# dan-lee-gh/monte-carlo-gp

Measured on AMD Instinct MI355X. Metric: race-simulations/sec (20 drivers, 60 laps), higher is better.
Workload: dtype f64

## Files before the change

### monte_carlo_gp_amd/csrc/mcgp_hip.hip

```cpp
#include "../../include/mcgp.h"
#include "params_build.h"
#include "race_kernel.hip.h"
#include "race_kernel_reg.hip.h"
#include "championship.hip.h"
#include "matchups.hip.h"
#include "resume.hip.h"

#define MCGP_FE_FN __host__ __device__ static inline
#include "frontend_exp.h"
#include "elo_update.h"
#include "normal53_table.h"

#include <hip/hip_runtime.h>

#include <cmath>
#include <cstdio>
#include <cstdlib>
#include <algorithm>
#include <cstring>
#include <mutex>
#include <new>
#include <string>
#include <vector>

// ... 191 lines not shown
    c.champ_keys_bytes = c.champ_bytes = 0;
    if (c.d_match) (void)hipFree(c.d_match);
    c.d_match = nullptr;
    c.match_bytes = 0;
    if (c.d_resume) (void)hipFree(c.d_resume);
    c.d_resume = nullptr;
    c.resume_bytes = 0;
    c.batch_bytes = c.batch_retire_bytes = 0;
    for (auto &t : c.timer) {
        if (t.start) (void)hipEventDestroy(t.start);
        if (t.stop) (void)hipEventDestroy(t.stop);
        if (t.d_ticket) (void)hipFree(t.d_ticket);
        if (t.d_retire) (void)hipFree(t.d_retire);
        t = DeviceCtx::Timer{};
    }
    c.last_timer = -1;
    c.d_hist = nullptr;
    c.d_grid = c.d_order1 = c.d_orders = nullptr;
    c.d_orders_bytes = 0;
}

int init_ctx_body(int device, DeviceCtx &c)
{
    HIP_TRY(hipSetDevice(device));
    hipDeviceProp_t prop;
    HIP_TRY(hipGetDeviceProperties(&prop, device));
    c.cu_count = prop.multiProcessorCount;
    c.lds_per_block = prop.sharedMemPerBlock;
    if (const char *e = std::getenv("MCGP_LDS_PER_BLOCK")) {
        const unsigned long long v = std::strtoull(e, nullptr, 10);
        if (v >= 16384 && v < c.lds_per_block) c.lds_per_block = (size_t)v;
    }
    for (auto &sl : c.slot) {
        HIP_TRY(hipMalloc(&sl.dev, sizeof(mcgp::KParams)));
        HIP_TRY(hipHostMalloc(&sl.host, sizeof(mcgp::KParams)));
        HIP_TRY(hipEventCreateWithFlags(&sl.uploaded, hipEventDisableTiming));
    }
    HIP_TRY(hipMalloc(&c.d_hist, sizeof(unsigned long long) * MCGP_MAX_CARS * MCGP_MAX_CARS));
    HIP_TRY(hipMalloc(&c.d_grid, MCGP_MAX_CARS));
    HIP_TRY(hipMalloc(&c.d_order1, MCGP_MAX_CARS));
    HIP_TRY(hipMalloc(&c.d_fe_in, sizeof(double) * 4 * MCGP_MAX_CARS));
    HIP_TRY(hipMalloc(&c.d_fe_pen, sizeof(int32_t) * MCGP_MAX_CARS));
    HIP_TRY(hipMalloc(&c.d_fe_out, sizeof(double) * MCGP_MAX_CARS * MCGP_MAX_CARS));
    HIP_TRY(hipMalloc(&c.d_norm53, sizeof(mcgp_normal53_table_bits)));
    HIP_TRY(hipMemcpy(c.d_norm53, mcgp_normal53_table_bits, sizeof(mcgp_normal53_table_bits), hipMemcpyHostToDevice));
    HIP_TRY(hipFuncSetAttribute(reinterpret_cast<const void *>(&mcgp::race_kernel),
                                hipFuncAttributeMaxDynamicSharedMemorySize, (int)c.lds_per_block));
    HIP_TRY(hipFuncSetAttribute(reinterpret_cast<const void *>(&mcgp::race_resume_kernel),
                                hipFuncAttributeMaxDynamicSharedMemorySize, (int)c.lds_per_block));
    return MCGP_OK;
}

int ensure_ctx_locked(int device, DeviceCtx &c)
{
    if (c.ready) return MCGP_OK;
    const int rc = init_ctx_body(device, c);
    if (rc != MCGP_OK) {
        release_ctx(c);
        return rc;
    }
    c.ready = true;
    return MCGP_OK;
}

int build_params(const mcgp_config *cfg, const mcgp_drivers *drv, const double *grid_probs, uint32_t n,
                 mcgp::KParams *kp)
{
    const char *err = "";
// ... 51 lines not shown
        MCGP_REG_SIZES(X)
#undef X
        default: return nullptr;
    }
}

KernelFn select_small_kernel(uint32_t n)
{
    switch (n) {
#define X(N_) case N_: return &mcgp::race_kernel_reg<N_, mcgp::kSmallBlockWaves>;
        MCGP_REG_SIZES(X)
#undef X
        default: return nullptr;
    }
}

KernelFn select_kernel(const mcgp::KParams &kp, bool *is_reg)
{
    *is_reg = false;
    const uint32_t n = (uint32_t)kp.n;
    const char *force = std::getenv("MCGP_FORCE_GENERIC");
    if (force && force[0] == '1') return &mcgp::race_kernel;
    if (!mcgp::reg_kernel_serves(kp)) return &mcgp::race_kernel;
    switch (n) {
#define X(N_) case N_: *is_reg = true; return &mcgp::race_kernel_reg<N_>;
        MCGP_REG_SIZES(X)
#undef X
        default: return &mcgp::race_kernel;
    }
}

void launch_geometry(const DeviceCtx &c, uint32_t n, bool is_reg, KernelFn kernel, uint64_t n_sims, uint32_t *grid,
                     uint32_t *block, uint32_t *lds, int reg_waves = 0 ,
                     bool wide = false , int total_laps = 0)
{
    int reg_cap = 8;
    {
        hipFuncAttributes attr;
        if (hipFuncGetAttributes(&attr, reinterpret_cast<const void *>(kernel)) == hipSuccess && attr.numRegs > 0) {
            const int alloc = ((attr.numRegs + 7) / 8) * 8;
            int per_simd = 512 / alloc;
            if (per_simd > 8) per_simd = 8;
            if (per_simd < 1) per_simd = 1;
            reg_cap = 4 * per_simd;
        }
    }
    int waves = 1, blocks_per_cu = 1;
    size_t bytes = 0;
    if (is_reg) {
        waves = reg_waves ? reg_waves : mcgp::reg_block_waves((int)n);
        bytes = wide ? mcgp::wide_launch_lds_bytes((int)n, waves, total_laps)
                     : mcgp::shared_lds_bytes_reg((int)n) + (size_t)waves * 64 * mcgp::per_thread_lds_bytes_reg((int)n);
    } else {
        const size_t per_wave = 64 * mcgp::per_thread_lds_bytes((int)n);
        waves = (int)((c.lds_per_block - mcgp::kSharedTableBytes) / per_wave);
        if (waves > 8) waves = 8;
        if (waves < 1) waves = 1;
        uint32_t threads = (uint32_t)waves * 64u;
        if (n_sims < threads) threads = (uint32_t)(((n_sims + 63) / 64) * 64);
        if (threads == 0) threads = 64;
        waves = (int)(threads / 64);
        bytes = mcgp::kSharedTableBytes + (size_t)threads * mcgp::per_thread_lds_bytes((int)n);
    }
    blocks_per_cu = (int)(c.lds_per_block / bytes);
    if (blocks_per_cu * waves > reg_cap) blocks_per_cu = reg_cap / waves;
    if (blocks_per_cu < 1) blocks_per_cu = 1;
    const uint32_t threads = (uint32_t)waves * 64u;
    const uint64_t n_batches = (n_sims + threads - 1) / threads;
    uint64_t g = (uint64_t)c.cu_count * (uint64_t)blocks_per_cu;
    if (g > n_batches) g = n_batches;
    if (g < 1) g = 1;
    *grid = (uint32_t)g;
    *block = threads;
    *lds = (uint32_t)bytes;
}

uint64_t max_sims_per_launch()
{
    uint64_t cap = 0xFFFFFE00ull;
    if (const char *e = std::getenv("MCGP_MAX_SIMS_PER_LAUNCH")) {
        const unsigned long long v = std::strtoull(e, nullptr, 10);
        if (v >= 1 && v < cap) cap = v;
    }
    return cap;
// ... 56 lines not shown

int launch(DeviceCtx &c, const mcgp::KParams &kp, uint64_t n_sims, uint64_t sim_offset, uint64_t seed,
           hipStream_t stream, unsigned long long *d_hist, uint8_t *d_orders, const uint8_t *d_fixed_grid,
           const FrontEnd &fe = FrontEnd())
{
    if (n_sims == 0) return MCGP_OK;
    bool is_reg = false;
    KernelFn kernel = select_kernel(kp, &is_reg);
    WideKernelFn wide = nullptr;
    if (kp.wide) {
        wide = select_wide_kernel((uint32_t)kp.n);
        if (!wide || !mcgp::reg_kernel_serves(kp))
            return fail(MCGP_E_BAD_ARG, "deviates = MCGP_DEVIATES_53 serves the problems the register kernel takes "
                                        "(reg_kernel_serves: lap times clear of zero, overtake_delta >= 0)");
        HIP_TRY(hipFuncSetAttribute(reinterpret_cast<const void *>(wide), hipFuncAttributeMaxDynamicSharedMemorySize,
                                    (int)c.lds_per_block));
        is_reg = true;
        kernel = nullptr;
    }
    DeviceCtx::Slot *sl = nullptr;
    if (!fe.on)
        for (auto &cand : c.slot)
            if (cand.used && cand.shareable && std::memcmp(cand.host, &kp, sizeof(kp)) == 0) { sl = &cand; break; }
    if (!sl) {
        sl = &c.slot[c.next_slot];
        c.next_slot = (c.next_slot + 1) % kParamSlots;
        if (sl->used)
            for (auto &rd : sl->reader)
                if (rd.live) {
                    HIP_TRY(hipEventSynchronize(rd.done));
                    rd.live = false;
                }
        std::memcpy(sl->host, &kp, sizeof(kp));
        sl->used = true;
        sl->shareable = !fe.on;
        HIP_TRY(hipMemcpyAsync(sl->dev, sl->host, sizeof(kp), hipMemcpyHostToDevice, stream));
        if (fe.on) {
            hipLaunchKernelGGL(grid_probs_kernel, dim3(1), dim3(mcgp::kMaxCars), 0, stream, c.d_fe_in, c.d_fe_pen,
                               (int)kp.n, sl->dev->grid_probs);
            HIP_TRY(hipGetLastError());
        }
        HIP_TRY(hipEventRecord(sl->uploaded, stream));
        sl->upload_stream = stream;
    } else if (sl->upload_stream != stream) {
        HIP_TRY(hipStreamWaitEvent(stream, sl->uploaded, 0));
    }
    int ti = -1;
    {
        const int rc = claim_timer(c, stream, &ti);
        if (rc != MCGP_OK) return rc;
    }
    c.timer[ti].seq = ++c.timer_seq;
    if (!c.timer[ti].d_ticket) return fail(MCGP_E_HIP, "no work counter for this stream");
    HIP_TRY(hipEventRecord(c.timer[ti].start, stream));
    const uint64_t cap = max_sims_per_launch();
    uint32_t grid = 0, block = 0, lds = 0;
    bool small_shape = false;
    auto resource_error = [](hipError_t e) {
        return e == hipErrorOutOfMemory || e == hipErrorInvalidValue || e == hipErrorLaunchOutOfResources ||
               e == hipErrorInvalidConfiguration;
    };
    for (uint64_t done = 0; done < n_sims; done += cap) {
        const uint64_t m = (n_sims - done) < cap ? (n_sims - done) : cap;
        for (;;) {
            KernelFn k = kernel;
            if (small_shape) {
                k = select_small_kernel((uint32_t)kp.n);
                if (!k) return fail(MCGP_E_HIP, "no small-block instantiation for this field size");
            }
            launch_geometry(c, (uint32_t)kp.n, is_reg, wide ? reinterpret_cast<KernelFn>(wide) : k, m, &grid, &block, &lds,
                            wide ? mcgp::wide_block_waves(kp.n) : small_shape ? mcgp::kSmallBlockWaves : 0, wide != nullptr,
                            kp.total_laps);
            const bool may_shrink = is_reg && !wide && !small_shape;
            if (may_shrink && lds > c.lds_per_block) {
                small_shape = true;
                continue;
            }
            if (lds > c.lds_per_block)
                return fail(MCGP_E_HIP, "the kernel's smallest block needs " + std::to_string(lds) + " bytes of LDS, the device offers " +
                                            std::to_string(c.lds_per_block) + " per block");
            if (is_reg && !wide) {
                const hipError_t e = hipFuncSetAttribute(reinterpret_cast<const void *>(k),
                                                         hipFuncAttributeMaxDynamicSharedMemorySize, (int)lds);
                if (e != hipSuccess) {
                    (void)hipGetLastError();
                    if (may_shrink && resource_error(e)) { small_shape = true; continue; }
                    return fail(MCGP_E_HIP, std::string("hipFuncSetAttribute(dynamic LDS): ") + hipGetErrorString(e));
                }
            }
            const uint64_t unit = is_reg ? 64u : block;
            const uint64_t n_batches = (m + unit - 1) / unit;
            if (is_reg) {
                HIP_TRY(hipMemsetAsync(c.timer[ti].d_ticket, 0, sizeof(uint32_t), stream));
                const size_t want = mcgp::reg_retire_ws_bytes(kp.n, (size_t)grid * block);
                if (want > c.timer[ti].retire_bytes) {
                    if (c.timer[ti].d_retire) {
                        HIP_TRY(hipStreamSynchronize(stream));
                        (void)hipFree(c.timer[ti].d_retire);
                    }
                    c.timer[ti].d_retire = nullptr;
                    c.timer[ti].retire_bytes = 0;
                    HIP_TRY(hipMalloc(&c.timer[ti].d_retire, want));
                    c.timer[ti].retire_bytes = want;
                }
            }
// ... 942 lines not shown
```

### monte_carlo_gp_amd/csrc/params_build.h

```cpp
#pragma once
#include "../../include/mcgp.h"
#include "normal_table.h"
#include "race_common.hip.h"

#include <cmath>
#include <cstring>

namespace mcgp {

inline uint64_t threshold(double p)
{
    if (!(p > 0.0)) return 0;
    const double x = p * 4294967296.0;
    if (x >= 4294967296.0) return 4294967296ull;
    return (uint64_t)std::ceil(x);
}

inline uint64_t threshold53(double p)
{
    if (!(p > 0.0)) return 0;
    const double x = p * 9007199254740992.0;
    if (x >= 9007199254740992.0) return 9007199254740992ull;
    return (uint64_t)std::ceil(x);
}
// ... 48 lines not shown
        if (cfg->comp_optimal_laps[c] < 0 || cfg->comp_optimal_laps[c] > 50000)
            { *err = "comp_optimal_laps out of range"; return MCGP_E_BAD_ARG; }
    }
    for (uint32_t d = 0; d < n; ++d) {
        const double deg = drv->tire_deg[d];
        kp->base_pace[d] = drv->base_pace[d];
        kp->factor[d] = deg > 0 ? deg / 0.05 : 1.0;
        kp->tire_deg[d] = deg;
        kp->variance[d] = drv->variance[d];
        kp->t_dnf1[d] = threshold(drv->team_dnf[d] * 4.0);
        kp->t_dnf[d] = threshold(drv->lap_dnf[d]);
        kp->t53_dnf1[d] = threshold53(drv->team_dnf[d] * 4.0);
        kp->q64_dnf[d] = survival64(drv->lap_dnf[d]);
        const double pit_deg = drv->tire_deg_pit[d];
        for (int c = 0; c < 5; ++c) {
            int opt = cfg->comp_optimal_laps[c];
            if (pit_deg > 0.05) opt = (int)((double)opt * 0.85);
            else if (pit_deg < 0.02) opt = (int)((double)opt * 1.1);
            kp->opt_laps[d * kCompStride + c] = (uint16_t)opt;
        }
    }
    if (grid_probs)
        for (uint32_t d = 0; d < n; ++d)
            for (uint32_t s = 0; s < n; ++s) {
                const double p = grid_probs[(size_t)d * n + s];
                if (!(p >= 0.0)) { *err = "grid_probs has a negative or NaN entry"; return MCGP_E_BAD_ARG; }
                kp->grid_probs[(size_t)d * n + s] = p;
            }
    static_assert(sizeof(mcgp_normal_table_bits) == sizeof(kp->normal_bits), "normal table size");
    std::memcpy(kp->normal_bits, mcgp_normal_table_bits, sizeof(kp->normal_bits));
    return MCGP_OK;
}

}
```

### monte_carlo_gp_amd/csrc/race_common.hip.h

```cpp
#pragma once
#include <hip/hip_runtime.h>
#include <stdint.h>

namespace mcgp {

constexpr int kMaxCars = 32;
constexpr int kNormalRows = 448;
constexpr int kNormal53Rows = 784;
constexpr int kNormal53RowBytes = 64;
constexpr int kCompStride = 8;

constexpr uint32_t kPurposeGrid = 0u << 16;
constexpr uint32_t kPurposeEvent = 1u << 16;
constexpr uint32_t kPurposeCar = 2u << 16;
constexpr uint32_t kPurposeOvt = 3u << 16;
constexpr uint32_t kPurposeRetire = 4u << 16;

__host__ __device__ inline uint32_t retire_next_threshold(uint32_t S, uint32_t q)
{
    return (uint32_t)(((uint64_t)S * (uint64_t)q) >> 32);
}
__host__ __device__ inline uint32_t draw_retirement_lap(uint32_t w, uint64_t t, int L)
{
    if (t == 0ull) return 0u;
// ... 1 lines not shown
    uint32_t S = q;
    for (int k = 2; k <= L; ++k) {
        if (!(w < S)) return (uint32_t)k;
        S = retire_next_threshold(S, q);
    }
    return 0u;
}
__host__ __device__ inline uint32_t draw_retirement_lap_after(uint32_t w, uint64_t t, int k, int L)
{
    const uint32_t r = draw_retirement_lap(w, t, L - k + 1);
    return r == 0u ? 0u : (uint32_t)(k - 1) + r;
}

struct KParams {
    int32_t n, total_laps, track, pop_sh, pop_mh, pad0;
    double pit_loss, overtake_delta, drs_delta, dirty_thr, dirty_pen;
    double overtake_delta_31;
    uint64_t t_red, t_sc, t_vsc, t_vsc_tire;
    double comp_deg[kCompStride], comp_delta[kCompStride];
    double base_pace[kMaxCars];
    double factor[kMaxCars];
    double tire_deg[kMaxCars];
    double variance[kMaxCars];
    uint64_t t_dnf1[kMaxCars];
    uint64_t t_dnf[kMaxCars];
    uint16_t opt_laps[kMaxCars * kCompStride];
    double grid_probs[kMaxCars * kMaxCars];
    uint32_t normal_bits[kNormalRows * 4];
    int32_t wide, pad1;
    uint64_t t53_red, t53_sc, t53_vsc, t53_vsc_tire;
    uint64_t t53_dnf1[kMaxCars];
    uint64_t q64_dnf[kMaxCars];
};

constexpr size_t kSharedTableBytes =
    kNormalRows * 16
    + 4 * kMaxCars * 8
    + 2 * kMaxCars * 8
    + kMaxCars * kCompStride * 2
    + 2 * kCompStride * 8
    + kMaxCars * kMaxCars * 4;
__host__ __device__ constexpr size_t per_thread_lds_bytes(int n) { return (size_t)n * (8 + 8 + 4 + 1 + 2); }

__device__ __forceinline__ uint32_t xor3_key(uint32_t a, uint32_t b, uint32_t key)
{
#if defined(__HIP_DEVICE_COMPILE__)
    uint32_t r;
    asm("v_bitop3_b32 %0, %1, %2, %3 bitop3:0x96" : "=v"(r) : "v"(a), "v"(b), "s"(key));
    return r;
#else
    return a ^ b ^ key;
#endif
}

__device__ __forceinline__ void philox4x32_10(uint32_t c0, uint32_t c1, uint32_t c2, uint32_t c3,
                                              uint32_t k0, uint32_t k1,
                                              uint32_t &o0, uint32_t &o1, uint32_t &o2, uint32_t &o3)
{
#pragma unroll
    for (int r = 0; r < 10; ++r) {
        const uint64_t p0 = (uint64_t)0xD2511F53u * c0;
        const uint64_t p1 = (uint64_t)0xCD9E8D57u * c2;
        const uint32_t n0 = xor3_key((uint32_t)(p1 >> 32), c1, k0);
        const uint32_t n2 = xor3_key((uint32_t)(p0 >> 32), c3, k1);
        c1 = (uint32_t)p1;
        c3 = (uint32_t)p0;
// ... 93 lines not shown
```

### monte_carlo_gp_amd/csrc/race_isa.hip.h

```cpp
#ifndef MCGP_RACE_ISA_H
#define MCGP_RACE_ISA_H
#include <hip/hip_runtime.h>

namespace mcgp {

__device__ __forceinline__ void minmax_f64(double a, double b, double &lo, double &hi)
{
    asm("v_min_f64 %0, %1, %2" : "=v"(lo) : "v"(a), "v"(b));
    asm("v_max_f64 %0, %1, %2" : "=v"(hi) : "v"(a), "v"(b));
}

__device__ __forceinline__ double max_f64(double a, double b)
{
    double r;
    asm("v_max_f64 %0, %1, %2" : "=v"(r) : "v"(a), "v"(b));
    return r;
}

__device__ __forceinline__ double max_abs_f64(double a, double b)
{
    double r;
    asm("v_max_f64 %0, |%1|, %2" : "=v"(r) : "v"(a), "v"(b));
    return r;
}
// ... 223 lines not shown
            "v_ceil_f64 %[t], %[dl]\n\t"
            "v_cvt_u32_f64 %[thr], %[t]\n\t"
            "v_min_u32 %[thr], 0x80000000, %[thr]\n\t"
            "v_add_u32 %[next], %[stride], %[row]\n\t"
            "v_cndmask_b32 %[thr], 0, %[thr], vcc\n\t"
            "v_cndmask_b32 %[next], %[row], %[next], vcc"
            : [t] "=&v"(t), [thr] "=&v"(thr), [next] "=&v"(next)
            : [dl] "v"(dl), [od] "s"(od), [row] "v"(row), [stride] "n"(STRIDE)
            : "vcc");
    } else {
        asm("v_cmp_lt_f64 vcc, %[od], %[dl]\n\t"
            "v_cvt_u32_f64 %[thr], %[dl]\n\t"
            "v_add_u32 %[next], %[stride], %[row]\n\t"
            "v_min_u32 %[thr], 0x80000000, %[thr]\n\t"
            "v_cndmask_b32 %[next], %[row], %[next], vcc\n\t"
            "v_cndmask_b32 %[thr], 0, %[thr], vcc"
            : [thr] "=&v"(thr), [next] "=&v"(next)
            : [dl] "v"(dl), [od] "s"(od), [row] "v"(row), [stride] "n"(STRIDE)
            : "vcc");
    }
}

#define MCGP_LDS __attribute__((address_space(3)))
template <typename T>
__device__ __forceinline__ T lds_ld(uint32_t addr)
{
    return *reinterpret_cast<const MCGP_LDS T *>(addr);
}
template <typename T>
__device__ __forceinline__ void lds_st(uint32_t addr, T v)
{
    *reinterpret_cast<MCGP_LDS T *>(addr) = v;
}
__device__ __forceinline__ void lds_or_u32(uint32_t addr, uint32_t bits)
{
    (void)__hip_atomic_fetch_or(reinterpret_cast<MCGP_LDS uint32_t *>(addr), bits, __ATOMIC_RELAXED, __HIP_MEMORY_SCOPE_WAVEFRONT);
}
__device__ __forceinline__ float4 lds_ld_float4(uint32_t addr)
{
    typedef float v4f __attribute__((ext_vector_type(4)));
    const v4f v = *reinterpret_cast<const MCGP_LDS v4f *>(addr);
    return make_float4(v.x, v.y, v.z, v.w);
}
struct f64x2 {
    double x, y;
};
__device__ __forceinline__ f64x2 lds_ld_f64x2(uint32_t addr)
{
    typedef double v2d __attribute__((ext_vector_type(2)));
    const v2d v = *reinterpret_cast<const MCGP_LDS v2d *>(addr);
    return f64x2{v.x, v.y};
}
__device__ __forceinline__ void lds_st_f64x2(uint32_t addr, double a, double b)
{
    typedef double v2d __attribute__((ext_vector_type(2)));
    v2d v;
    v.x = a;
    v.y = b;
    *reinterpret_cast<MCGP_LDS v2d *>(addr) = v;
}
__device__ __forceinline__ void lds_st_u32x4(uint32_t addr, uint32_t a, uint32_t b, uint32_t c, uint32_t d)
{
    typedef uint32_t v4u __attribute__((ext_vector_type(4)));
    v4u v;
    v.x = a; v.y = b; v.z = c; v.w = d;
    *reinterpret_cast<MCGP_LDS v4u *>(addr) = v;
// ... 74 lines not shown
```

### monte_carlo_gp_amd/csrc/race_kernel_reg.hip.h

```cpp
#pragma once
#include "race_common.hip.h"
#include "race_isa.hip.h"
#include "sort_networks.h"

#include <utility>

#ifndef MCGP_STAT
#define MCGP_STAT(what, value)
#endif
#ifndef MCGP_TRACE_PASS
#define MCGP_TRACE_PASS(sim, lap, pass, n_cand)
#endif
#ifndef MCGP_COOPERATIVE_EVENTS
#define MCGP_COOPERATIVE_EVENTS 1
#endif
#ifndef MCGP_GRID_EXACT
#define MCGP_GRID_EXACT 0
#endif
#ifndef MCGP_WIDE_EXACT
#define MCGP_WIDE_EXACT 0
#endif
#ifndef MCGP_WIDE_TIE_SHIFT
#define MCGP_WIDE_TIE_SHIFT 0
#endif
// ... 34 lines not shown
constexpr size_t kLdsReserve = 256;
__host__ __device__ constexpr int block_shape_rank(int w) { return (w % 4 == 0 ? 0 : 100) + (w <= 8 ? 2 * (8 - w) : w - 8); }
__host__ __device__ constexpr int reg_block_waves(int n)
{
    const int cap = 4 * reg_min_waves(n);
    int best = 0, waves = 1;
    for (int w = 1; w <= kMaxBlockWaves; ++w) {
        int b = (int)((kLdsPerCu - kLdsReserve) / (shared_lds_bytes_reg(n) + (size_t)w * 64 * per_thread_lds_bytes_reg(n)));
        if (b * w > cap) b = cap / w;
        if (b < 1) continue;
        if (b * w > best || (b * w == best && block_shape_rank(w) < block_shape_rank(waves))) { best = b * w; waves = w; }
    }
    return waves;
}

__host__ __device__ constexpr size_t reg_retire_ws_bytes(int n, size_t lanes) { return (size_t)(n + 1) * lanes * 4; }

constexpr int kWideLdsRowsMax = 32 * 16;
constexpr int kNorm53LdsStride = 80;
__host__ __device__ constexpr size_t wide_fixed_lds_bytes(int n, int waves)
{
    return shared_lds_bytes_reg(n) - (size_t)kNormalRows * 16 + (size_t)waves * 64 * per_thread_lds_bytes_reg(n);
}
__host__ __device__ constexpr int wide_lds_rows(int n, int waves)
{
    const size_t fixed = wide_fixed_lds_bytes(n, waves);
    const size_t room = kLdsPerCu - kLdsReserve > fixed ? kLdsPerCu - kLdsReserve - fixed : 0;
    int rows = (int)(room / (size_t)kNorm53LdsStride) / 16 * 16;
    return rows > kWideLdsRowsMax ? kWideLdsRowsMax : rows;
}
__host__ __device__ constexpr size_t wide_lds_bytes(int n, int waves)
{
    return wide_fixed_lds_bytes(n, waves) + (size_t)wide_lds_rows(n, waves) * kNorm53LdsStride;
}
__host__ __device__ constexpr size_t wide_chain_bytes(int n, int total_laps)
{
    return total_laps >= 2 ? (size_t)(total_laps - 1) * (size_t)((n + 3) & ~3) * 8 : 0;
}
__host__ __device__ constexpr size_t wide_launch_lds_bytes(int n, int waves, int total_laps)
{
    const size_t base = wide_lds_bytes(n, waves), chain = wide_chain_bytes(n, total_laps);
    return base + chain + kLdsReserve <= kLdsPerCu ? base + chain : base;
}
template <int N, int WAVES = reg_block_waves(N), bool WIDE = false>
struct RegGeo {
    static constexpr int kWaves = WAVES;
    static constexpr bool kWide = WIDE;
    static constexpr int B = 64 * kWaves;
    static constexpr uint32_t oDrvA = 0;
    static constexpr uint32_t oDrvB = oDrvA + N * 16;
    static constexpr uint32_t oIc = oDrvB + (kMaxCars + N) * 16;
    static constexpr uint32_t oComp = oIc + ((kNumCompounds - 1) * kMaxCars + N) * 16;
    static constexpr uint32_t oDrs = oComp + kCompStride * 16;
    static constexpr uint32_t oPit = oDrs + 16;
    static constexpr uint32_t oDrsB = oDrs + 32;
    static constexpr uint32_t oLut = oDrsB + 32;
    static constexpr uint32_t oNorm = oLut + 128;
    static constexpr uint32_t oHist = oNorm + (WIDE ? 0 : kNormalRows * 16);
    static_assert(WIDE || oNorm >= kNormalRowBias * 16, "the inverse-normal rows are addressed through a base 48 rows before the table");
    static constexpr uint32_t oGrid = oHist + (uint32_t)align16((size_t)N * N * 4);
    static constexpr uint32_t oW = oGrid + (uint32_t)align16((size_t)N * N * 8);
    static constexpr uint32_t oLast = oW + (uint32_t)kWordRows * B * 4;
    static constexpr uint32_t oNorm53 = oLast + (uint32_t)N * B * 8;
    static constexpr int kNorm53Rows = WIDE ? wide_lds_rows(N, WAVES) : 0;
    static constexpr int kNorm53First = kNormal53Rows - kNorm53Rows;
    static constexpr uint32_t kBytes = oNorm53 + (uint32_t)kNorm53Rows * (uint32_t)kNorm53LdsStride;
    static constexpr uint32_t oChain = kBytes;
    static constexpr uint32_t kChainStride = (uint32_t)((N + 3) & ~3) * 8u;
    __host__ __device__ static constexpr bool chain_fits(int total_laps)
    {
        return WIDE && total_laps >= 2 && kBytes + wide_chain_bytes(N, total_laps) + kLdsReserve <= kLdsPerCu;
    }
    static_assert(oW == shared_lds_bytes_reg(N) - (WIDE ? (size_t)kNormalRows * 16 : 0) && oLast % 8 == 0, "LDS map");
    static_assert(oW % 16 == 0 && oNorm53 % 16 == 0, "the event handler parks fields with 16-byte LDS accesses (ds_write_b128 / ds_read_b128); table rows are read 16 bytes at a time");
    static_assert(kBytes == (WIDE ? wide_lds_bytes(N, WAVES) : per_thread_lds_bytes_reg(N) * B + shared_lds_bytes_reg(N)), "LDS map");
    static_assert(kBytes + kLdsReserve <= kLdsPerCu, "block does not fit LDS");
    static_assert(oLast < 65536, "row bases must fit the DS immediate offset");
};
constexpr int kWideMinLdsRows = 14 * 16;
__host__ __device__ constexpr int wide_block_waves(int n)
{
    if (n <= 22) {
        for (int w = 12; w > 8; --w)
            if (wide_fixed_lds_bytes(n, w) + kLdsReserve <= kLdsPerCu && wide_lds_rows(n, w) >= kWideMinLdsRows) return w;
    }
    int w = 8;
    while (w > 1 && wide_fixed_lds_bytes(n, w) + kLdsReserve > kLdsPerCu) --w;
    return w;
}
__host__ __device__ constexpr int wide_min_waves(int n) { return wide_block_waves(n) > 8 ? 3 : 2; }
template <int N>
using WideGeo = RegGeo<N, wide_block_waves(N), true>;

template <int N>
struct SortNetwork {
    int a[N * 8];
    int b[N * 8];
    int step[N * 8];
    int n;
    int ga[N * 8];
    int gn[N * 8];
    int n_groups;
    constexpr SortNetwork() : a{}, b{}, step{}, n(0), ga{}, gn{}, n_groups(0)
    {
        const SortNetworkTable *table = nullptr;
// ... 240 lines not shown
        const double f = kp.base_pace[d] - var * z_max + eff_min * 2047.0;
        floor_ = f < floor_ ? f : floor_;
        if (!(f == f)) return f;
    }
    floor_ = floor_ + cdelta_min - 110.0 * 0.03 - (kp.drs_delta > 0 ? kp.drs_delta : 0.0) +
             (kp.dirty_pen < 0 ? kp.dirty_pen : 0.0) - 0.5 * 1.5 * z_max;
    return floor_;
}

__host__ __device__ inline bool reg_kernel_serves(const KParams &kp)
{
    if (!(kp.overtake_delta >= 0.0)) return false;
    const double big = 0x1p900, tiny = 0x1p-900;
    auto scalable = [&](double x) { return x == 0.0 || (x > -big && x < big && (x >= tiny || x <= -tiny)); };
    for (int d = 0; d < kp.n; ++d) {
        if (!scalable(kp.base_pace[d]) || !scalable(kp.tire_deg[d])) return false;
        for (int c = 0; c < 5; ++c)
            if (!scalable(kp.comp_deg[c] * kp.factor[d])) return false;
    }
    return reg_time_floor(kp) >= kRegTimeFloor;
}

template <int N, class G = RegGeo<N>>
__device__ __forceinline__ void reg_load_tables(const KParams *__restrict__ P, unsigned char *smem, uint32_t tid,
                                                const double *__restrict__ norm53 = nullptr)
{
    constexpr int B = G::B;
    uint32_t *s_hist = reinterpret_cast<uint32_t *>(smem + G::oHist);
    double *t_grid = reinterpret_cast<double *>(smem + G::oGrid);
    if constexpr (G::kWide) {
        double *t53 = reinterpret_cast<double *>(smem + G::oNorm53);
        for (uint32_t i = tid; i < (uint32_t)G::kNorm53Rows * 8u; i += B)
            t53[(i >> 3) * (kNorm53LdsStride / 8) + (i & 7u)] = norm53[(uint32_t)G::kNorm53First * 8u + i];
        if (G::chain_fits(P->total_laps)) {
            for (uint32_t d = tid; d < G::kChainStride / 8u; d += B) {
                const uint64_t q = d < (uint32_t)N ? P->q64_dnf[d] : 0ull;
                uint64_t S = q;
                for (int k = 2; k <= P->total_laps; ++k) {
                    *reinterpret_cast<uint64_t *>(smem + G::oChain + (uint32_t)(k - 2) * G::kChainStride + d * 8u) = S;
                    S = __umul64hi(S, q);
                }
            }
        }
    } else {
        float4 *t_norm = reinterpret_cast<float4 *>(smem + G::oNorm);
        for (uint32_t i = tid; i < (uint32_t)kNormalRows * 4; i += B)
            reinterpret_cast<uint32_t *>(t_norm)[i] = P->normal_bits[i];
    }
    for (uint32_t d = tid; d < (uint32_t)N; d += B) {
        double *a = reinterpret_cast<double *>(smem + G::oDrvA + d * 16);
        double *b = reinterpret_cast<double *>(smem + G::oDrvB + d * 16);
        const double qnan = __builtin_nan("");
        a[0] = P->variance[d];
        a[1] = P->base_pace[d];
        b[0] = P->base_pace[d] * 2147483648.0;
        b[1] = P->tire_deg[d] * 32768.0;
        b[2 * kMaxCars] = qnan;
        b[2 * kMaxCars + 1] = qnan;
    }
    if (tid < 2) {
        *reinterpret_cast<double *>(smem + G::oDrs + tid * k3Drs) = tid ? P->drs_delta : 0.0;
        *reinterpret_cast<double *>(smem + G::oDrsB + tid * k3Drs) = tid ? P->drs_delta * 2147483648.0 : 0.0;
        *reinterpret_cast<double *>(smem + G::oPit + tid * 8u) = tid ? P->pit_loss : 0.0;
    }
    for (uint32_t i = tid; i < (uint32_t)kNumCompounds * N; i += B) {
        const uint32_t c = i / N, d = i % N;
        unsigned char *r = smem + G::oIc + (c * kMaxCars + d) * 16;
        *reinterpret_cast<double *>(r) = (P->comp_deg[c] * P->factor[d]) * kAgeFieldUnit;
        *reinterpret_cast<uint32_t *>(r + 8) = (uint32_t)P->opt_laps[d * kCompStride + c] << 16;
        *reinterpret_cast<uint32_t *>(r + 12) = 0u;
    }
    for (uint32_t i = tid; i < 32u; i += B)
        *reinterpret_cast<uint32_t *>(smem + G::oLut + i * 4) =
            pit_rule_word(P->track, (int)(i >> 3), i & 7u, (uint32_t)P->pop_sh, (uint32_t)P->pop_mh);
    for (uint32_t c = tid; c < (uint32_t)kCompStride; c += B) {
        double *r = reinterpret_cast<double *>(smem + G::oComp + c * 16);
// ... 351 lines not shown
        network_sort<N>(cum, pk);
        update_positions_reg<N>(cum, pk, false, dirty_thr);

        constexpr uint32_t kNoKey = 0x7FFFu;
        auto retirements_after = [&](const uint32_t *ws, uint32_t after) -> uint32_t {
            const uint32_t n_out = ws[(size_t)N * ws_stride];
            uint32_t k1 = kNoKey, k2 = kNoKey, left = 0u;
#pragma unroll 1
            for (uint32_t k = 0; k < n_out; ++k) {
                const uint32_t e = ws[(size_t)k * ws_stride];
                if (e > after) {
                    ++left;
                    const uint32_t hi = e > k1 ? e : k1;
                    k1 = e < k1 ? e : k1;
                    k2 = hi < k2 ? hi : k2;
                }
            }
            return k1 | (k2 << 16) | (left > 2u ? 0x80000000u : 0u);
        };
        uint32_t next_out;
        {
            uint32_t tid_w = tid;
            pin(tid_w);
            uint32_t *retire_ws = retire_ws_base + ws_first_lane + tid_w;
            uint32_t n_out = 0u, k1 = kNoKey, k2 = kNoKey;
#pragma unroll 1
            for (int d0 = 0; d0 < N; d0 += 4) {
                uint32_t rw[4];
                philox4x32_10(c0, c1, 0u, kPurposeRetire | (uint32_t)(d0 >> 2), seed_lo, seed_hi, rw[0], rw[1], rw[2], rw[3]);
                uint32_t survived[4];
                if constexpr (WIDE) {
                    uint32_t rx[4];
                    philox4x32_10(c0, c1, 0u, kPurposeRetire | kCompanion | (uint32_t)(d0 >> 2), seed_lo, seed_hi, rx[0], rx[1], rx[2], rx[3]);
                    uint64_t Q[4], q64[4], S64[4];
#pragma unroll
                    for (int j = 0; j < 4; ++j) {
                        Q[j] = ((uint64_t)rw[j] << 32) | ((uint64_t)(rx[j] >> 11) << 11);
                        q64[j] = d0 + j < N ? P->q64_dnf[d0 + j] : 0ull;
                        S64[j] = q64[j];
                        survived[j] = 0u;
                    }
                    if (G::chain_fits(L)) {
                        uint32_t a = G::oChain + (uint32_t)d0 * 8u;
#pragma unroll 1
                        for (int k = 2; k <= L; ++k) {
#pragma unroll
                            for (int j = 0; j < 4; ++j) survived[j] += Q[j] < lds_ld<uint64_t>(a + 8u * j) ? 1u : 0u;
                            a += G::kChainStride;
                        }
                    } else {
#pragma unroll 1
                    for (int k = 2; k <= L; ++k) {
#pragma unroll
                        for (int j = 0; j < 4; ++j) {
                            survived[j] += Q[j] < S64[j] ? 1u : 0u;
                            S64[j] = __umul64hi(S64[j], q64[j]);
                        }
                    }
                    }
                } else {
                uint32_t q[4], S[4];
#pragma unroll
                for (int j = 0; j < 4; ++j) {
                    const uint64_t t = d0 + j < N ? P->t_dnf[d0 + j] : 0ull;
                    q[j] = (uint32_t)(4294967296ull - t);
                    S[j] = q[j];
                    survived[j] = 0u;
                }
#pragma unroll 1
                for (int k = 2; k <= L; ++k) {
#pragma unroll
                    for (int j = 0; j < 4; ++j) {
                        survived[j] += rw[j] < S[j] ? 1u : 0u;
                        S[j] = retire_next_threshold(S[j], q[j]);
                    }
                }
                }
#pragma unroll
                for (int j = 0; j < 4; ++j) {
                    const int d = d0 + j;
                    if (d >= N) continue;
                    if (P->t_dnf[d] == 0ull) continue;
                    const uint32_t out_lap = 2u + survived[j];
                    if (out_lap <= (uint32_t)L) {
                        const uint32_t key = (out_lap << 5) | (uint32_t)d;
                        if (n_out == 2u) {
                            retire_ws[0] = k1;
                            retire_ws[(size_t)ws_stride] = k2;
                        }
                        if (n_out >= 2u) retire_ws[(size_t)n_out * ws_stride] = key;
                        ++n_out;
// ... 379 lines not shown
                            for (int j = 0; j < H; ++j) {
                                if (h + j < N) {
                                    const uint32_t id16 = pk_slot16(pk[h + j]);
                                    const f64x2 bd = lds_ld_f64x2(G::oDrvB + id16);
                                    pb[j] = bd.x;
                                    pd[j] = bd.y;
                                    pa[j] = lds_ld<double>(G::oDrsB + (pk[h + j] & k3Drs));
                                }
                            }
#pragma unroll
                            for (int j = 0; j < H; ++j) {
                                const int i = h + j;
                                if (i < N) {
                                    const double pace = pb[j] + (double)(pk[i] & k3AgeMask) * pd[j];
                                    if (i > 0) {
                                        const double dl = (pace_prev - pace) + pa[j];
                                        uint32_t next;
                                        ovt_threshold<(uint32_t)(B * 4), !WIDE>(dl, od31, row, thr[i], next);
                                        ow[i] = lds_ld<uint32_t>(G::oW + row);
                                        row = next;
                                    }
                                    pace_prev = pace;
                                }
                            }
                        }
                        thr[0] = 0u;
                        ow[0] = 0u;
                    }
                    const uint32_t words_end = row - tid4;
                    MCGP_STAT(0 + pass, words_end != 0u);
                    if (words_end == 0u) break;
                    n_attempts = words_end / (uint32_t)(B * 4);
                    if constexpr (WIDE) {
                        bool tie = false;
#pragma unroll
                        for (int i = 1; i < N; ++i) tie |= ((ow[i] ^ thr[i]) >> MCGP_WIDE_TIE_SHIFT) == 0u;
                        MCGP_STAT(11, tie);
                        if (__builtin_expect(MCGP_ANY(tie || MCGP_WIDE_EXACT || words_end > (uint32_t)(kWordRows * B * 4)), 0)) {
                            const uint32_t hits = wide_pass_exact();
#pragma unroll
                            for (int i = 1; i < N; ++i) {
                                thr[i] = (hits >> i) & 1u;
                                ow[i] = 0u;
                            }
                        }
                    } else if (__builtin_expect(MCGP_ANY(words_end > (uint32_t)(kWordRows * B * 4)), 0)) {
                        uint32_t cand = 0u;
#pragma unroll
                        for (int i = 1; i < N; ++i) cand |= thr[i] != 0u ? (1u << i) : 0u;
                        uint32_t hits = 0u, rest = cand;
#pragma unroll 1
                        for (int chunk = 0; rest != 0u; ++chunk) {
                            uint32_t m = rest;
#pragma unroll 1
                            for (int k = 0; k < kWordRows && m != 0u; ++k) m &= m - 1u;
                            const uint32_t cur = rest & ~m;
#pragma unroll 1
                            for (int b = 0; b < 2; ++b) {
                                uint32_t o0, o1, o2, o3;
                                philox4x32_10(c0l, c1l, (uint32_t)lap, kPurposeOvt | (uint32_t)(8 * pass + 2 * chunk + b), k0l,
                                              k1l, o0, o1, o2, o3);
                                lds_st<uint32_t>(w_row(4 * b + 0), o0);
                                lds_st<uint32_t>(w_row(4 * b + 1), o1);
                                lds_st<uint32_t>(w_row(4 * b + 2), o2);
                                lds_st<uint32_t>(w_row(4 * b + 3), o3);
                            }
                            uint32_t h = 0u;
#pragma unroll
                            for (int i = 1; i < N; ++i) {
// ... 167 lines not shown
```

Measured before the change: 148.1 million.

## Precompute survival-threshold table on host and read it via scalar loads

Moves the per-driver survival threshold chain (repeated 64-bit products of q) from a per-block LDS build into a host-built table placed right after the kernel parameter block and uploaded with it. The wide retirement loop now reads four thresholds at once with uniform scalar (constant address space) loads instead of LDS reads or per-lap multiply-high, which frees LDS that the old chain occupied. It also rewrites the tie check as a running min of XOR values compared once against a threshold. The trade-off is a larger host-to-device parameter upload and host work per new parameter set.

```diff
diff --git a/monte_carlo_gp_amd/csrc/mcgp_hip.hip b/monte_carlo_gp_amd/csrc/mcgp_hip.hip
--- a/monte_carlo_gp_amd/csrc/mcgp_hip.hip
+++ b/monte_carlo_gp_amd/csrc/mcgp_hip.hip
@@ -247,8 +247,8 @@
         if (v >= 16384 && v < c.lds_per_block) c.lds_per_block = (size_t)v;
     }
     for (auto &sl : c.slot) {
-        HIP_TRY(hipMalloc(&sl.dev, sizeof(mcgp::KParams)));
-        HIP_TRY(hipHostMalloc(&sl.host, sizeof(mcgp::KParams)));
+        HIP_TRY(hipMalloc(&sl.dev, sizeof(mcgp::KParams) + mcgp::kSurv64MaxBytes));
+        HIP_TRY(hipHostMalloc(&sl.host, sizeof(mcgp::KParams) + mcgp::kSurv64MaxBytes));
         HIP_TRY(hipEventCreateWithFlags(&sl.uploaded, hipEventDisableTiming));
     }
     HIP_TRY(hipMalloc(&c.d_hist, sizeof(unsigned long long) * MCGP_MAX_CARS * MCGP_MAX_CARS));
@@ -366,7 +366,7 @@
 
 void launch_geometry(const DeviceCtx &c, uint32_t n, bool is_reg, KernelFn kernel, uint64_t n_sims, uint32_t *grid,
                      uint32_t *block, uint32_t *lds, int reg_waves = 0 ,
-                     bool wide = false , int total_laps = 0)
+                     bool wide = false )
 {
     int reg_cap = 8;
     {
@@ -383,7 +383,7 @@
     size_t bytes = 0;
     if (is_reg) {
         waves = reg_waves ? reg_waves : mcgp::reg_block_waves((int)n);
-        bytes = wide ? mcgp::wide_launch_lds_bytes((int)n, waves, total_laps)
+        bytes = wide ? mcgp::wide_lds_bytes((int)n, waves)
                      : mcgp::shared_lds_bytes_reg((int)n) + (size_t)waves * 64 * mcgp::per_thread_lds_bytes_reg((int)n);
     } else {
         const size_t per_wave = 64 * mcgp::per_thread_lds_bytes((int)n);
@@ -506,9 +506,11 @@
                     rd.live = false;
                 }
         std::memcpy(sl->host, &kp, sizeof(kp));
+        const size_t surv = kp.wide ? mcgp::surv64_bytes(kp.n, kp.total_laps) : 0;
+        if (surv) mcgp::build_surv64(kp, const_cast<uint64_t *>(mcgp::surv64_of(sl->host)));
         sl->used = true;
         sl->shareable = !fe.on;
-        HIP_TRY(hipMemcpyAsync(sl->dev, sl->host, sizeof(kp), hipMemcpyHostToDevice, stream));
+        HIP_TRY(hipMemcpyAsync(sl->dev, sl->host, sizeof(kp) + surv, hipMemcpyHostToDevice, stream));
         if (fe.on) {
             hipLaunchKernelGGL(grid_probs_kernel, dim3(1), dim3(mcgp::kMaxCars), 0, stream, c.d_fe_in, c.d_fe_pen,
                                (int)kp.n, sl->dev->grid_probs);
@@ -543,8 +545,7 @@
                 if (!k) return fail(MCGP_E_HIP, "no small-block instantiation for this field size");
             }
             launch_geometry(c, (uint32_t)kp.n, is_reg, wide ? reinterpret_cast<KernelFn>(wide) : k, m, &grid, &block, &lds,
-                            wide ? mcgp::wide_block_waves(kp.n) : small_shape ? mcgp::kSmallBlockWaves : 0, wide != nullptr,
-                            kp.total_laps);
+                            wide ? mcgp::wide_block_waves(kp.n) : small_shape ? mcgp::kSmallBlockWaves : 0, wide != nullptr);
             const bool may_shrink = is_reg && !wide && !small_shape;
             if (may_shrink && lds > c.lds_per_block) {
                 small_shape = true;
diff --git a/monte_carlo_gp_amd/csrc/params_build.h b/monte_carlo_gp_amd/csrc/params_build.h
--- a/monte_carlo_gp_amd/csrc/params_build.h
+++ b/monte_carlo_gp_amd/csrc/params_build.h
@@ -104,4 +104,18 @@
     return MCGP_OK;
 }
 
+static_assert(kMaxLaps == MCGP_MAX_LAPS, "survival table size");
+inline void build_surv64(const KParams &kp, uint64_t *out)
+{
+    const int stride = surv64_stride(kp.n);
+    for (int d = 0; d < stride; ++d) {
+        const uint64_t q = d < kp.n ? kp.q64_dnf[d] : 0ull;
+        uint64_t S = q;
+        for (int k = 2; k <= kp.total_laps; ++k) {
+            out[(size_t)(k - 2) * (size_t)stride + (size_t)d] = S;
+            S = (uint64_t)(((unsigned __int128)S * q) >> 64);
+        }
+    }
 }
+
+}
diff --git a/monte_carlo_gp_amd/csrc/race_common.hip.h b/monte_carlo_gp_amd/csrc/race_common.hip.h
--- a/monte_carlo_gp_amd/csrc/race_common.hip.h
+++ b/monte_carlo_gp_amd/csrc/race_common.hip.h
@@ -57,6 +57,16 @@
     uint64_t t53_dnf1[kMaxCars];
     uint64_t q64_dnf[kMaxCars];
 };
+
+__host__ __device__ constexpr int surv64_stride(int n) { return (n + 3) & ~3; }
+__host__ __device__ constexpr size_t surv64_bytes(int n, int total_laps)
+{
+    return total_laps >= 2 ? (size_t)(total_laps - 1) * (size_t)surv64_stride(n) * 8 : 0;
+}
+constexpr int kMaxLaps = 1000;
+constexpr size_t kSurv64MaxBytes = surv64_bytes(kMaxCars, kMaxLaps);
+static_assert(sizeof(KParams) % 16 == 0, "the survival table behind the parameter block is read 8 and 16 bytes at a time");
+__host__ __device__ inline const uint64_t *surv64_of(const KParams *P) { return reinterpret_cast<const uint64_t *>(P + 1); }
 
 constexpr size_t kSharedTableBytes =
     kNormalRows * 16
diff --git a/monte_carlo_gp_amd/csrc/race_isa.hip.h b/monte_carlo_gp_amd/csrc/race_isa.hip.h
--- a/monte_carlo_gp_amd/csrc/race_isa.hip.h
+++ b/monte_carlo_gp_amd/csrc/race_isa.hip.h
@@ -279,6 +279,17 @@
 {
     *reinterpret_cast<MCGP_LDS T *>(addr) = v;
 }
+struct u64x4 {
+    uint64_t v[4];
+};
+__device__ __forceinline__ u64x4 sload_u64x4(const uint64_t *p)
+{
+#if defined(__HIP_DEVICE_COMPILE__)
+    return *reinterpret_cast<const __attribute__((address_space(4))) u64x4 *>(reinterpret_cast<uintptr_t>(p));
+#else
+    return *reinterpret_cast<const u64x4 *>(p);
+#endif
+}
 __device__ __forceinline__ void lds_or_u32(uint32_t addr, uint32_t bits)
 {
     (void)__hip_atomic_fetch_or(reinterpret_cast<MCGP_LDS uint32_t *>(addr), bits, __ATOMIC_RELAXED, __HIP_MEMORY_SCOPE_WAVEFRONT);
diff --git a/monte_carlo_gp_amd/csrc/race_kernel_reg.hip.h b/monte_carlo_gp_amd/csrc/race_kernel_reg.hip.h
--- a/monte_carlo_gp_amd/csrc/race_kernel_reg.hip.h
+++ b/monte_carlo_gp_amd/csrc/race_kernel_reg.hip.h
@@ -90,15 +90,6 @@
 __host__ __device__ constexpr size_t wide_lds_bytes(int n, int waves)
 {
     return wide_fixed_lds_bytes(n, waves) + (size_t)wide_lds_rows(n, waves) * kNorm53LdsStride;
-}
-__host__ __device__ constexpr size_t wide_chain_bytes(int n, int total_laps)
-{
-    return total_laps >= 2 ? (size_t)(total_laps - 1) * (size_t)((n + 3) & ~3) * 8 : 0;
-}
-__host__ __device__ constexpr size_t wide_launch_lds_bytes(int n, int waves, int total_laps)
-{
-    const size_t base = wide_lds_bytes(n, waves), chain = wide_chain_bytes(n, total_laps);
-    return base + chain + kLdsReserve <= kLdsPerCu ? base + chain : base;
 }
 template <int N, int WAVES = reg_block_waves(N), bool WIDE = false>
 struct RegGeo {
@@ -123,12 +114,6 @@
     static constexpr int kNorm53Rows = WIDE ? wide_lds_rows(N, WAVES) : 0;
     static constexpr int kNorm53First = kNormal53Rows - kNorm53Rows;
     static constexpr uint32_t kBytes = oNorm53 + (uint32_t)kNorm53Rows * (uint32_t)kNorm53LdsStride;
-    static constexpr uint32_t oChain = kBytes;
-    static constexpr uint32_t kChainStride = (uint32_t)((N + 3) & ~3) * 8u;
-    __host__ __device__ static constexpr bool chain_fits(int total_laps)
-    {
-        return WIDE && total_laps >= 2 && kBytes + wide_chain_bytes(N, total_laps) + kLdsReserve <= kLdsPerCu;
-    }
     static_assert(oW == shared_lds_bytes_reg(N) - (WIDE ? (size_t)kNormalRows * 16 : 0) && oLast % 8 == 0, "LDS map");
     static_assert(oW % 16 == 0 && oNorm53 % 16 == 0, "the event handler parks fields with 16-byte LDS accesses (ds_write_b128 / ds_read_b128); table rows are read 16 bytes at a time");
     static_assert(kBytes == (WIDE ? wide_lds_bytes(N, WAVES) : per_thread_lds_bytes_reg(N) * B + shared_lds_bytes_reg(N)), "LDS map");
@@ -435,16 +420,6 @@
         double *t53 = reinterpret_cast<double *>(smem + G::oNorm53);
         for (uint32_t i = tid; i < (uint32_t)G::kNorm53Rows * 8u; i += B)
             t53[(i >> 3) * (kNorm53LdsStride / 8) + (i & 7u)] = norm53[(uint32_t)G::kNorm53First * 8u + i];
-        if (G::chain_fits(P->total_laps)) {
-            for (uint32_t d = tid; d < G::kChainStride / 8u; d += B) {
-                const uint64_t q = d < (uint32_t)N ? P->q64_dnf[d] : 0ull;
-                uint64_t S = q;
-                for (int k = 2; k <= P->total_laps; ++k) {
-                    *reinterpret_cast<uint64_t *>(smem + G::oChain + (uint32_t)(k - 2) * G::kChainStride + d * 8u) = S;
-                    S = __umul64hi(S, q);
-                }
-            }
-        }
     } else {
         float4 *t_norm = reinterpret_cast<float4 *>(smem + G::oNorm);
         for (uint32_t i = tid; i < (uint32_t)kNormalRows * 4; i += B)
@@ -862,31 +837,21 @@
                 if constexpr (WIDE) {
                     uint32_t rx[4];
                     philox4x32_10(c0, c1, 0u, kPurposeRetire | kCompanion | (uint32_t)(d0 >> 2), seed_lo, seed_hi, rx[0], rx[1], rx[2], rx[3]);
-                    uint64_t Q[4], q64[4], S64[4];
+                    uint64_t Q[4];
 #pragma unroll
                     for (int j = 0; j < 4; ++j) {
                         Q[j] = ((uint64_t)rw[j] << 32) | ((uint64_t)(rx[j] >> 11) << 11);
-                        q64[j] = d0 + j < N ? P->q64_dnf[d0 + j] : 0ull;
-                        S64[j] = q64[j];
                         survived[j] = 0u;
                     }
-                    if (G::chain_fits(L)) {
-                        uint32_t a = G::oChain + (uint32_t)d0 * 8u;
-#pragma unroll 1
-                        for (int k = 2; k <= L; ++k) {
-#pragma unroll
-                            for (int j = 0; j < 4; ++j) survived[j] += Q[j] < lds_ld<uint64_t>(a + 8u * j) ? 1u : 0u;
-                            a += G::kChainStride;
-                        }
-                    } else {
-#pragma unroll 1
+                    const KParams *Ps = P;
+                    pin_ptr(Ps);
+                    const uint64_t *S = surv64_of(Ps) + d0;
+#pragma unroll 2
                     for (int k = 2; k <= L; ++k) {
-#pragma unroll
-                        for (int j = 0; j < 4; ++j) {
-                            survived[j] += Q[j] < S64[j] ? 1u : 0u;
-                            S64[j] = __umul64hi(S64[j], q64[j]);
-                        }
-                    }
+                        const u64x4 s = sload_u64x4(S);
+#pragma unroll
+                        for (int j = 0; j < 4; ++j) survived[j] += Q[j] < s.v[j] ? 1u : 0u;
+                        S += surv64_stride(N);
                     }
                 } else {
                 uint32_t q[4], S[4];
@@ -1332,9 +1297,13 @@
                     if (words_end == 0u) break;
                     n_attempts = words_end / (uint32_t)(B * 4);
                     if constexpr (WIDE) {
-                        bool tie = false;
-#pragma unroll
-                        for (int i = 1; i < N; ++i) tie |= ((ow[i] ^ thr[i]) >> MCGP_WIDE_TIE_SHIFT) == 0u;
+                        uint32_t near_min = 0xFFFFFFFFu;
+#pragma unroll
+                        for (int i = 1; i < N; ++i) {
+                            const uint32_t x = ow[i] ^ thr[i];
+                            near_min = x < near_min ? x : near_min;
+                        }
+                        const bool tie = near_min < (1u << MCGP_WIDE_TIE_SHIFT);
                         MCGP_STAT(11, tie);
                         if (__builtin_expect(MCGP_ANY(tie || MCGP_WIDE_EXACT || words_end > (uint32_t)(kWordRows * B * 4)), 0)) {
                             const uint32_t hits = wide_pass_exact();
```

New measurement: 148.1 million, median of 6. Within noise of the previous version (-0.0%).
